# 4m4n5/CLIP-Lite

Hardware: AMD Instinct MI355X
Metric: image-caption pairs/sec (global batch) — ResNet-50+BERT bs1024, 1/2/4/8 MI355X (higher is better)
Workload: dtype bf16; 1 GPU; resnet50 + BERT-base(12L) + JSD-MI heads/priors, per-GPU batch 128, 224x224 images, 30-token captions, dropout 0.1 + prior noise on, clip 10 + SGD(0.9, wd 1e-4) + Lookahead(5, 0.5); global_batch=128, parallelism=dp1

## Files before the change

clip-lite_amd/csrc/conv_patch.hip:

```cpp
#include "igemm_wide.h"
#include "wide_api.h"
#include <type_traits>
#include "stem_bn.h"

using namespace clite;

#ifndef CLITE_PATCH_WGS
#define CLITE_PATCH_WGS 256
#endif

namespace {

constexpr int PC = 64;
constexpr int PIXB = PC * 2;
constexpr int NTAP = 9;
constexpr int WBYTES = NTAP * PC * PIXB;
constexpr int MAXPIX = 344;
constexpr int PBYTES = MAXPIX * PIXB;
constexpr int NPI = MAXPIX / 8;
constexpr int NPW = (NPI + 7) / 8;
constexpr int EPITCH = PC * 4 + 16;
constexpr int HALF = 128;
static_assert(HALF * EPITCH <= PBYTES, "a half of the accumulator tile fits a patch buffer");
static_assert(WBYTES + 2 * PBYTES <= 160 * 1024, "LDS budget");
// ... 265 lines not shown
  a.x = x; a.xbytes = (uint32_t)((size_t)c.N * c.H * c.W * PC * 2);
  a.w = w; a.wbytes = (uint32_t)(NTAP * PC * PC * 2);
  a.N = c.N; a.H = c.H; a.W = c.W; a.R = R;
  a.strips_per_img = (c.H + R - 1) / R;
  a.nstrips = c.N * a.strips_per_img;
  a.flip = dgrad ? 1 : 0;
  const int grid = a.nstrips < CLITE_PATCH_WGS ? a.nstrips : CLITE_PATCH_WGS;
  const int per = (a.nstrips + grid - 1) / grid;
  const int g2 = (a.nstrips + per - 1) / per;
  if (form == 0) hipLaunchKernelGGL(conv3x3_patch_kernel<0>, dim3(g2), dim3(512), 0, st, a, ep, per);
  else hipLaunchKernelGGL(conv3x3_patch_kernel<1>, dim3(g2), dim3(512), 0, st, a, ep, per);
  return (int)hipGetLastError();
}

namespace {

constexpr int WG_DYPIX = 256;
constexpr int WG_XPIX = 376;
constexpr int WG_DYB = WG_DYPIX * PIXB, WG_XB = WG_XPIX * PIXB, WG_STAGE = WG_DYB + WG_XB;
constexpr int WG_NI_DY = WG_DYPIX / 8, WG_NI_X = WG_XPIX / 8;
constexpr int WG_NW_DY = (WG_NI_DY + 7) / 8, WG_NW_X = (WG_NI_X + 7) / 8;
constexpr int WG_OUT = NTAP * PC * PC;
static_assert(2 * WG_STAGE <= 160 * 1024, "LDS budget");

struct WgradPatchArgs {
  const void* dy;
  const void* x;
  uint32_t bytes;
  int N, H, W, R;
  int strips_per_img, nstrips;
  float* ws;
};

DEV int wg_frag_base(int pix0, int x0, int lane) {
  const int x = x0 + 16 * ((lane >> 4) & 1) + 4 * (lane & 3);
  const int pix = pix0 + 8 * (lane >> 5) + ((lane >> 2) & 3);
  const int b = x * 2;
  return pix * PIXB + ((((b >> 6) ^ (pix >> 1)) & 1) << 6) + (b & 63);
}
DEV bf16x8 wg_frag_at(const char* p) {
  const s16x4 lo = lds_read_tr16(p);
  const s16x4 hi = lds_read_tr16(p + 4 * PIXB);
  union { s16x4 v[2]; bf16x8 h; } u;
  u.v[0] = lo; u.v[1] = hi;
  return u.h;
}

__global__ __launch_bounds__(512) void conv3x3_wgrad_patch_kernel(WgradPatchArgs a, int strips_per_wg) {
  __shared__ __attribute__((aligned(1024))) char smem[2 * WG_STAGE];
  const int tid = threadIdx.x;
  const int lane = tid & 63;
  const int wave = wave_uniform(tid >> 6);
  const int W1 = a.W + 1;

  int s_begin = blockIdx.x * strips_per_wg, s_end = s_begin + strips_per_wg;
  if (s_end > a.nstrips) s_end = a.nstrips;

  const rsrc_t rdy = make_rsrc(a.dy, a.bytes), rx = make_rsrc(a.x, a.bytes);
  int d_rel[WG_NW_DY], d_row[WG_NW_DY], x_rel[WG_NW_X], x_row[WG_NW_X];
#pragma unroll
  for (int k = 0; k < WG_NW_DY; ++k) {
    const int i = wave + 8 * k;
    const int pix = i * 8 + (lane >> 3);
    const int oy = pix / W1, ox = pix - oy * W1;
    const int chunk = (lane & 7) ^ (((pix >> 1) & 1) << 2);
    const bool ok = i < WG_NI_DY && ox < a.W && oy < a.R;
    d_row[k] = ok ? oy : -1;
    d_rel[k] = (oy * a.W + ox) * PC + chunk * 8;
  }
#pragma unroll
  for (int k = 0; k < WG_NW_X; ++k) {
    const int i = wave + 8 * k;
    const int pix = i * 8 + (lane >> 3);
    const int pr = pix / W1, pc = pix - pr * W1;
    const int chunk = (lane & 7) ^ (((pix >> 1) & 1) << 2);
    const bool ok = i < WG_NI_X && pc >= 1 && pc <= a.W && pr <= a.R + 1;
    x_row[k] = ok ? pr : -1;
    x_rel[k] = ((pr - 1) * a.W + (pc - 1)) * PC + chunk * 8;
  }
  auto issue = [&](int strip, char* dst) {
// ... 298 lines not shown
```

clip-lite_amd/csrc/gemm_group.hip:

```cpp
#include "igemm_wide.h"
#include "det.h"
#include <string.h>
#include <algorithm>
#include <vector>

using namespace clite;

namespace {

constexpr int GBK = 32;
#ifndef CLITE_GROUP_KCHUNK
#define CLITE_GROUP_KCHUNK 256
#endif
constexpr int KCHUNK = CLITE_GROUP_KCHUNK;

template <class LA, class LB>
struct GroupItem {
  LA la;
  LB lb;
  float* out;
  int ldc, M, N, ktiles, chunk;
  int zeroed;
  const float* row_scale;
  const float* sa;
  const float* sb;
};
struct WgEntry { uint32_t item, tile_m, tile_n, kchunk; };

template <class CFG, class LA, class LB, int NSTAGE>
__global__ __launch_bounds__(256) void igemm_group_kernel(const GroupItem<LA, LB>* __restrict__ items, const WgEntry* __restrict__ map) {
  typedef bf16 T;
  constexpr int BM = CFG::BM, BN = CFG::BN, BK = CFG::BK;
  constexpr int RM = CFG::RM, RN = CFG::RN;
  constexpr int STAGE = LA::BYTES + LB::BYTES;
  constexpr int LOADS_PER_TILE = LA::NI + LB::NI;
  __shared__ __attribute__((aligned(1024))) char smem[NSTAGE * STAGE];

  const int tid = threadIdx.x;
  const int lane = tid & 63;
  const int wave = wave_uniform(tid >> 6);
  const int wm0 = (wave / CFG::WAVES_N) * CFG::WM;
  const int wn0 = (wave % CFG::WAVES_N) * CFG::WN;
  const WgEntry e = map[blockIdx.x];
  if (wave_uniform((int)e.item) < 0) return;
  const GroupItem<LA, LB>& it = items[wave_uniform((int)e.item)];
  const LA la = it.la;
  const LB lb = it.lb;
  const int M = it.M, N = it.N;
  const int m0 = wave_uniform((int)e.tile_m) * BM, n0 = wave_uniform((int)e.tile_n) * BN;
  const int t_begin = wave_uniform((int)e.kchunk) * it.chunk;
  int t_end = t_begin + it.chunk;
  if (t_end > it.ktiles) t_end = it.ktiles;

  typename LA::State sa;
  typename LB::State sb;
  la.init(sa, m0, wave, lane, t_begin);
  lb.init(sb, n0, wave, lane, t_begin);

  f32x16 acc[RM][RN];
#pragma unroll
  for (int i = 0; i < RM; ++i)
#pragma unroll
    for (int j = 0; j < RN; ++j)
#pragma unroll
      for (int r = 0; r < 16; ++r) acc[i][j][r] = 0.f;
  int aoff[RM][BK / 16], boff[RN][BK / 16];
#pragma unroll
  for (int ks = 0; ks < BK / 16; ++ks) {
#pragma unroll
    for (int i = 0; i < RM; ++i) aoff[i][ks] = LA::frag_off(wm0 + i * 32, ks, lane);
#pragma unroll
    for (int j = 0; j < RN; ++j) boff[j][ks] = LB::frag_off(wn0 + j * 32, ks, lane);
  }
#pragma unroll
  for (int pz = 0; pz < NSTAGE - 1; ++pz) {
    if (t_begin + pz < t_end) {
      DmaIssue<LA>::go(la, sa, smem + pz * STAGE, wave, lane, m0);
      DmaIssue<LB>::go(lb, sb, smem + pz * STAGE + LA::BYTES, wave, lane, n0);
// ... 242 lines not shown
    if (t + NSTAGE - 1 < t_end) {
      int nb = buf + NSTAGE - 1; if (nb >= NSTAGE) nb -= NSTAGE;
      WideIssue<LA>::go(la, sa, smem + nb * STAGE, wave, lane, m0);
      WideIssue<LB>::go(lb, sb, smem + nb * STAGE + LA::BYTES, wave, lane, n0);
    }
#pragma unroll
    for (int i = 0; i < RM; ++i)
#pragma unroll
      for (int j = 0; j < RN; ++j) acc[i][j] = mfma32x64_bf8_fp8(alo[i], ahi[i], blo[j], bhi[j], acc[i][j]);
    if (++buf == NSTAGE) buf = 0;
  }
  float* out = it.out;
  const int ldc = it.ldc;
  const float dq = it.sa[1] * it.sb[1];
  const float* rs = it.row_scale;
  const bool single = wave_uniform((int)(it.ktiles <= it.chunk && it.zeroed && !rs));
#pragma unroll
  for (int i = 0; i < RM; ++i)
#pragma unroll
    for (int j = 0; j < RN; ++j) {
      const int col = n0 + wn0 + j * 32 + (lane & 31);
#pragma unroll
      for (int r = 0; r < 16; ++r) {
        const int row = m0 + wm0 + i * 32 + (r & 3) + 8 * (r >> 2) + 4 * (lane >> 5);
        if (row < M && col < N) {
          float* q = out + (size_t)row * ldc + col;
          const float v = (rs ? acc[i][j][r] * rs[row] : acc[i][j][r]) * dq;
          if (single) *q = v; else atomic_add_f32(q, v);
        }
      }
    }
}

struct Plan { int M, N, Ktot, ktiles, chunk, nchunks, tm, tn; };
Plan plan(int M, int N, int Ktot, int BM, int BN, int bk = GBK, int kchunk = KCHUNK) {
  Plan p;
  p.M = M; p.N = N; p.Ktot = Ktot;
  p.ktiles = (Ktot + bk - 1) / bk;
  p.nchunks = (p.ktiles + kchunk - 1) / kchunk;
  p.chunk = (p.ktiles + p.nchunks - 1) / p.nchunks;
  p.nchunks = (p.ktiles + p.chunk - 1) / p.chunk;
  p.tm = (M + BM - 1) / BM; p.tn = (N + BN - 1) / BN;
  return p;
}

FastDiv fastdiv_make(uint32_t d) {
  FastDiv f;
  f.d = d;
  if (d <= 1) { f.mul = 0; f.shift = 0; f.d = 1; return f; }
  uint32_t l = 0;
  while ((1ull << l) < d) ++l;
  f.shift = l;
  f.mul = (uint32_t)((((1ull << l) - d) << 32) / d + 1);
  return f;
}
ConvGeom geom_fwd(const clite_conv& c) {
  ConvGeom g;
  g.H = c.H; g.W = c.W; g.C = c.C;
  g.sN = c.H * c.W * c.C; g.sH = c.W * c.C; g.sW = c.C;
  g.RH = c.Ho; g.RW = c.Wo; g.R = c.R; g.S = c.S; g.stride = c.stride; g.pad = c.pad; g.padw = c.pad;
  g.rows = c.N * c.Ho * c.Wo; g.concat = 0;
  g.div_hw = fastdiv_make(c.Ho * c.Wo);
  g.div_w = fastdiv_make(c.Wo);
  return g;
}

typedef TileCfg<128, 128, GBK, 64, 64> C128;
typedef TileCfg<64, 128, GBK, 64, 32> C64x128;
typedef TileCfg<128, 64, GBK, 32, 64> C128x64;
typedef DmaXCStrided<bf16, 128, GBK> XS128;
typedef DmaXCStrided<bf16, 64, GBK> XS64;
typedef DmaXCGather<bf16, 128, GBK> XG128;
typedef DmaXCGather<bf16, 64, GBK> XG64;
typedef WideCfg<256, 256, 128, 64, 1> W256;
typedef DmaXCStrided<bf16, 256, WIDE_BK, WIDE_NW> WS256;
typedef DmaXCGather<bf16, 256, WIDE_BK, WIDE_NW> WG256;
typedef DmaXCStrided<uint8_t, 256, WIDE_BK, WIDE_NW> FS256;
typedef DmaXCGather<uint8_t, 256, WIDE_BK, WIDE_NW> FG256;
constexpr int WKCHUNK = 128;
template <class CFG> struct GroupStages { static constexpr int n = 3; };
template <> struct GroupStages<W256> { static constexpr int n = 2; };

template <class CFG, class LA, class LB, bool WIDE = false, bool F8 = false>
struct Bucket {
  std::vector<GroupItem<LA, LB>> items;
  std::vector<Plan> plans;
  std::vector<WgEntry> map;
  void add(const LA& la, const LB& lb, float* out, int ldc, const Plan& p, int zeroed, const float* row_scale = nullptr, const float* sa = nullptr,
           const float* sb = nullptr) {
    GroupItem<LA, LB> it;
    it.la = la; it.lb = lb; it.out = out; it.ldc = ldc; it.M = p.M; it.N = p.N; it.ktiles = p.ktiles; it.chunk = p.chunk; it.zeroed = zeroed;
    it.row_scale = row_scale;
    it.sa = sa; it.sb = sb;
    items.push_back(it);
    plans.push_back(p);
  }
  static constexpr uint32_t NO_ITEM = 0xFFFFFFFFu;
  static constexpr int XCDS = 8, BUNDLE = WIDE ? 32 : 64;
  void build_map() {
    std::vector<uint32_t> order(items.size());
    for (uint32_t i = 0; i < order.size(); ++i) order[i] = i;
    std::stable_sort(order.begin(), order.end(), [&](uint32_t a, uint32_t b) { return plans[a].chunk > plans[b].chunk; });
    std::vector<WgEntry> per_xcd[XCDS];
    uint64_t load[XCDS] = {};
    for (uint32_t idx : order) {
      const Plan& p = plans[idx];
      const int tiles = p.tm * p.tn;
      for (int c = 0; c < p.nchunks; ++c) {
        int len = p.chunk;
        if ((c + 1) * p.chunk > p.ktiles) len = p.ktiles - c * p.chunk;
        for (int t0 = 0; t0 < tiles; t0 += BUNDLE) {
          const int t1 = t0 + BUNDLE < tiles ? t0 + BUNDLE : tiles;
          int x = 0;
          for (int k = 1; k < XCDS; ++k)
            if (load[k] < load[x]) x = k;
          for (int t = t0; t < t1; ++t) per_xcd[x].push_back(WgEntry{idx, (uint32_t)(t / p.tn), (uint32_t)(t % p.tn), (uint32_t)c});
          load[x] += (uint64_t)(t1 - t0) * (uint64_t)len;
        }
      }
    }
    size_t longest = 0;
    for (int k = 0; k < XCDS; ++k) longest = per_xcd[k].size() > longest ? per_xcd[k].size() : longest;
    map.assign(longest * XCDS, WgEntry{NO_ITEM, 0, 0, 0});
    for (int k = 0; k < XCDS; ++k)
      for (size_t j = 0; j < per_xcd[k].size(); ++j) map[j * XCDS + k] = per_xcd[k][j];
  }
  size_t n_wgs() const { return map.size(); }
  size_t item_bytes() const { return (items.size() * sizeof(GroupItem<LA, LB>) + 255) / 256 * 256; }
  size_t bytes() const { return item_bytes() + (n_wgs() * sizeof(WgEntry) + 255) / 256 * 256; }
  void stage(char* host, size_t off) {
    if (items.empty()) return;
    memcpy(host + off, items.data(), items.size() * sizeof(GroupItem<LA, LB>));
    memcpy(host + off + item_bytes(), map.data(), map.size() * sizeof(WgEntry));
  }
  int launch(char* dev, size_t off, hipStream_t st) const {
    if (items.empty()) return 0;
    if constexpr (F8)
      hipLaunchKernelGGL((igemm_group_fp8_kernel<CFG, LA, LB, 3>), dim3((unsigned)map.size()), dim3(512), 0, st,
                         (const GroupItem<LA, LB>*)(dev + off), (const WgEntry*)(dev + off + item_bytes()));
    else if constexpr (WIDE)
      hipLaunchKernelGGL((igemm_group_wide_kernel<CFG, LA, LB, GroupStages<CFG>::n>), dim3((unsigned)map.size()), dim3(512), 0, st,
                         (const GroupItem<LA, LB>*)(dev + off), (const WgEntry*)(dev + off + item_bytes()));
    else
      hipLaunchKernelGGL((igemm_group_kernel<CFG, LA, LB, 3>), dim3((unsigned)map.size()), dim3(256), 0, st,
                         (const GroupItem<LA, LB>*)(dev + off), (const WgEntry*)(dev + off + item_bytes()));
    return (int)hipGetLastError();
  }
};

bool fits32(size_t elems, size_t esize) { return elems * esize < 0xF0000000ull; }

}

bool clite_group_wide_enabled();

extern "C" int clite_wgrad_group(int dtype, const clite_wgrad_item* items, int n, void* ws_dev, void* ws_host, uint64_t ws_bytes, void* stream) {
  if (!items || n <= 0) return n == 0 ? 0 : -1;
  hipStream_t st = (hipStream_t)stream;
  if (dtype != CLITE_BF16 || clite::deterministic() || !ws_dev || !ws_host) {
    for (int i = 0; i < n; ++i) {
      const clite_wgrad_item& w = items[i];
      int rc;
      if (w.row_scale || (w.kind & 0xFF) == 2) return -1;
      if ((w.kind & ~(CLITE_WGRAD_NARROW | CLITE_WGRAD_ZEROED | CLITE_WGRAD_SHORTK)) == 0) {
        rc = clite_conv_wgrad(w.a, w.b, &w.cv, w.out, stream);
      } else {
        clite_epilogue ep = {};
        ep.out = w.out; ep.ldc = w.ldc; ep.out_f32 = 1; ep.atomic = 1; ep.alpha = 1.f;
        rc = clite_gemm_tn(w.a, w.lda, w.b, w.ldb, w.M, w.N, w.K, dtype, &ep, stream);
      }
      if (rc) return rc;
    }
    return 0;
  }
  Bucket<C128, XS128, XG128> conv_full;
  Bucket<C64x128, XS64, XG128> conv_fewk;
  Bucket<C128x64, XS128, XG64> conv_fewc;
  Bucket<C128, XS128, XS128> linear;
  Bucket<W256, WS256, WG256, true> conv_w256;
  Bucket<W256, WS256, WS256, true> linear_w256;
  Bucket<W256, FS256, FG256, true, true> conv_f8;
  const bool wide_all = clite_group_wide_enabled();
  for (int i = 0; i < n; ++i) {
    const clite_wgrad_item& w = items[i];
    if (!w.a || !w.b || !w.out) return -1;
    const bool wide = wide_all && !(w.kind & CLITE_WGRAD_NARROW);
    const int zeroed = (w.kind & CLITE_WGRAD_ZEROED) ? 1 : 0;
    const int kind = w.kind & ~(CLITE_WGRAD_NARROW | CLITE_WGRAD_ZEROED | CLITE_WGRAD_SHORTK);
    const int kc = (w.kind & CLITE_WGRAD_SHORTK) ? KCHUNK / 4 : KCHUNK, wkc = (w.kind & CLITE_WGRAD_SHORTK) ? WKCHUNK / 4 : WKCHUNK;
    if (kind == 0) {
      const clite_conv& c = w.cv;
      if (c.dtype != CLITE_BF16 || c.C % 8 || c.K % 8 || (c.R * c.S > 1 && (c.C % 32 || c.K % 32))) return -1;
      if (!fits32((size_t)c.N * c.H * c.W * c.C, 4) || !fits32((size_t)c.N * c.Ho * c.Wo * c.K, 4)) return -1;
      const int P = c.N * c.Ho * c.Wo, Ncols = c.R * c.S * c.C;
      const uint32_t yb = (uint32_t)((size_t)P * c.K * 2), xb = (uint32_t)((size_t)c.N * c.H * c.W * c.C * 2);
      if (wide && c.K >= 256 && Ncols >= 256) conv_w256.add(WS256{w.a, yb, c.K, c.K, P, 1}, WG256{w.b, xb, geom_fwd(c)}, w.out, Ncols, plan(c.K, Ncols, P, 256, 256, WIDE_BK, wkc), zeroed, w.row_scale);
      else if (c.K <= 64) conv_fewk.add(XS64{w.a, yb, c.K, c.K, P, 1}, XG128{w.b, xb, geom_fwd(c)}, w.out, Ncols, plan(c.K, Ncols, P, 64, 128, GBK, kc), zeroed, w.row_scale);
      else if (Ncols <= 64) conv_fewc.add(XS128{w.a, yb, c.K, c.K, P, 1}, XG64{w.b, xb, geom_fwd(c)}, w.out, Ncols, plan(c.K, Ncols, P, 128, 64, GBK, kc), zeroed, w.row_scale);
      else conv_full.add(XS128{w.a, yb, c.K, c.K, P, 1}, XG128{w.b, xb, geom_fwd(c)}, w.out, Ncols, plan(c.K, Ncols, P, 128, 128, GBK, kc), zeroed, w.row_scale);
    } else if (kind == 2) {
      const clite_conv& c = w.cv;
      if (!w.a_scales || !w.b_scales || c.dtype != CLITE_BF16 || c.C % 16 || c.K % 16 || (c.R * c.S > 1 && (c.C % 32 || c.K % 32))) return -1;
      if (!fits32((size_t)c.N * c.H * c.W * c.C, 1) || !fits32((size_t)c.N * c.Ho * c.Wo * c.K, 1)) return -1;
      const int P = c.N * c.Ho * c.Wo, Ncols = c.R * c.S * c.C;
      const uint32_t yb = (uint32_t)((size_t)P * c.K), xb = (uint32_t)((size_t)c.N * c.H * c.W * c.C);
      conv_f8.add(FS256{w.a, yb, c.K, c.K, P, 1}, FG256{w.b, xb, geom_fwd(c)}, w.out, Ncols, plan(c.K, Ncols, P, 256, 256, WIDE_BK, wkc), zeroed, w.row_scale, w.a_scales,
                  w.b_scales);
    } else if (kind == 1) {
      if (w.M <= 0 || w.N <= 0 || w.K <= 0 || w.M % 8 || w.N % 8 || w.lda % 8 || w.ldb % 8 || w.lda < w.M || w.ldb < w.N) return -1;
      if (!fits32((size_t)w.K * w.lda, 4) || !fits32((size_t)w.K * w.ldb, 4)) return -1;
      const uint32_t ab = (uint32_t)((((size_t)w.K - 1) * w.lda + w.M) * 2), bb = (uint32_t)((((size_t)w.K - 1) * w.ldb + w.N) * 2);
      if (wide && w.M >= 256 && w.N >= 256) linear_w256.add(WS256{w.a, ab, w.lda, w.M, w.K, 1}, WS256{w.b, bb, w.ldb, w.N, w.K, 1}, w.out, w.ldc, plan(w.M, w.N, w.K, 256, 256, WIDE_BK, wkc), zeroed, w.row_scale);
      else linear.add(XS128{w.a, ab, w.lda, w.M, w.K, 1}, XS128{w.b, bb, w.ldb, w.N, w.K, 1}, w.out, w.ldc, plan(w.M, w.N, w.K, 128, 128, GBK, kc), zeroed, w.row_scale);
    } else {
      return -1;
    }
  }
  conv_full.build_map(); conv_fewk.build_map(); conv_fewc.build_map(); linear.build_map();
  conv_w256.build_map(); linear_w256.build_map(); conv_f8.build_map();
  const size_t o0 = 0, o1 = o0 + conv_full.bytes(), o2 = o1 + conv_fewk.bytes(), o3 = o2 + conv_fewc.bytes(), o4 = o3 + linear.bytes(),
               o7 = o4 + conv_w256.bytes(), o8 = o7 + linear_w256.bytes(), need = o8 + conv_f8.bytes();
  if (need > ws_bytes) return -2;
  char* host = (char*)ws_host;
  char* dev = (char*)ws_dev;
  conv_full.stage(host, o0); conv_fewk.stage(host, o1); conv_fewc.stage(host, o2); linear.stage(host, o3);
  conv_w256.stage(host, o4); linear_w256.stage(host, o7); conv_f8.stage(host, o8);
  int rc = (int)hipMemcpyAsync(dev, host, need, hipMemcpyHostToDevice, st);
  if (rc) return rc;
  if ((rc = conv_f8.launch(dev, o8, st))) return rc;
  if ((rc = conv_w256.launch(dev, o4, st))) return rc;
  if ((rc = linear_w256.launch(dev, o7, st))) return rc;
  if ((rc = conv_full.launch(dev, o0, st))) return rc;
// ... 11 lines not shown
```

clip-lite_amd/csrc/igemm_dma.h:

```cpp
#ifndef CLITE_IGEMM_DMA_H
#define CLITE_IGEMM_DMA_H
#ifndef CLITE_ABLATE
#define CLITE_ABLATE 0
#endif
#ifndef CLITE_STAMP
#define CLITE_STAMP 0
#endif
#if CLITE_STAMP
__device__ unsigned long long clite_dbg[8 * 65536];
#define EPI_STAMP(i) do { if (threadIdx.x == 0 && blockIdx.x < 65536) clite_dbg[blockIdx.x * 8 + (i)] = __builtin_amdgcn_s_memrealtime(); } while (0)
#define STAMP(i) do { if (threadIdx.x == 0 && blockIdx.x < 65536) clite_dbg[blockIdx.x * 8 + (i)] = __builtin_amdgcn_s_memrealtime(); } while (0)
__shared__ unsigned long long clite_ph[8];
#define PHASE(i) do { if (threadIdx.x == 0) { unsigned long long n_ = __builtin_amdgcn_s_memrealtime(); clite_ph[i] += n_ - clite_ph[7]; clite_ph[7] = n_; } } while (0)
#define BN_EPI_PHASE(i) PHASE(i)
#else
#define STAMP(i) do {} while (0)
#define PHASE(i) do {} while (0)
#endif
#include "igemm.h"

namespace clite {

template <typename T, int ROWS, int BK, bool DGRAD>
struct DmaKC {
// ... 193 lines not shown
      int krow = (wave * NI + j) * RPI + lane / CPR;
      int c = (lane % CPR) ^ (xc_seg_xor<ROWB>(krow) << 2);
      int x = x0 + c * EPC;
      int rs = x / g.C;
      int ci = x - rs * g.C;
      st.r[j] = rs / g.S;
      st.s[j] = rs - st.r[j] * g.S;
      st.krow[j] = krow;
      st.xoff[j] = x < g.R * g.S * g.C ? ci : -1;
    }
    st.p0 = t_begin * BK;
  }
  DEV void issue(State& st, char* lds, int wave, int, int) const {
#pragma unroll
    for (int j = 0; j < NI; ++j) {
      int p = st.p0 + st.krow[j];
      bool v = st.xoff[j] >= 0 && p < g.rows;
      uint32_t n = fd_div(p, g.div_hw);
      uint32_t rem = p - n * g.div_hw.d;
      uint32_t ho = fd_div(rem, g.div_w);
      uint32_t wo = rem - ho * g.div_w.d;
      int hi = (int)ho * g.stride - g.pad + st.r[j];
      int wi = (int)wo * g.stride - g.padw + st.s[j];
      v = v && (unsigned)hi < (unsigned)g.H && (unsigned)wi < (unsigned)g.W;
      uint32_t off = v ? (uint32_t)((int)n * g.sN + hi * g.sH + wi * g.sW + st.xoff[j]) * (uint32_t)sizeof(T) : OOB_OFF;
      buf_load16_lds(st.rs_, off, lds + (wave * NI + j) * 1024);
    }
    st.p0 += BK;
  }
  DEV static int frag_off(int x0, int ks, int lane) { return L::frag_off(x0, ks, lane); }
  DEV static bf16x8 frag_at(const char* p) { return L::frag_at(p); }
  DEV static float frag32(const char* lds, int x0, int kk, int lane) { return L::frag32(lds, x0, kk, lane); }
  DEV static void frag8_f32(const char* lds, int x0, int lane, float (&v)[8]) { L::frag8_f32(lds, x0, lane, v); }
};

template <class L> struct DmaIssue {
  DEV static void go(const L& l, typename L::State& st, char* lds, int wave, int lane, int x0) { l.issue(st, lds, wave, lane, x0); }
};
template <typename T, int ROWS, int BK, bool D> struct DmaIssue<DmaKC<T, ROWS, BK, D>> {
  typedef DmaKC<T, ROWS, BK, D> L;
  DEV static void go(const L& l, typename L::State& st, char* lds, int wave, int, int) { l.issue(st, lds, wave); }
};

DEV void split_bf16x3(const float (&v)[8], bf16x8& hi, bf16x8& lo) {
#pragma unroll
  for (int e = 0; e < 8; ++e) {
    const bf16 h = f2bf(v[e]);
    hi[e] = h;
    lo[e] = f2bf(v[e] - bf2f(h));
  }
}
template <class CFG, class LA, class LB>
DEV void mma_tile_f32_split(const char* abuf, const char* bbuf, int wm0, int wn0, int lane, f32x16 (&acc)[CFG::RM][CFG::RN]) {
  constexpr int RM = CFG::RM, RN = CFG::RN;
  bf16x8 ah[RM], al[RM], bh[RN], bl[RN];
#pragma unroll
  for (int i = 0; i < RM; ++i) {
    float v[8];
    LA::frag8_f32(abuf, wm0 + i * 32, lane, v);
    split_bf16x3(v, ah[i], al[i]);
  }
#pragma unroll
  for (int j = 0; j < RN; ++j) {
    float v[8];
    LB::frag8_f32(bbuf, wn0 + j * 32, lane, v);
    split_bf16x3(v, bh[j], bl[j]);
// ... 530 lines not shown
```

clip-lite_amd/hip.py:

```python
import ctypes as C
import os

import torch

_HERE = os.path.dirname(os.path.abspath(__file__))
LIB_PATH = os.environ.get("CLITE_HIP_LIB") or os.path.join(_HERE, "lib", "libclite_hip.so")
ABI_VERSION = 12

BF16, F32 = 0, 1
ACT_NONE, ACT_RELU, ACT_GELU, ACT_TANH = 0, 1, 2, 3
DACT_RELU, DACT_GELU, DACT_TANH = 1, 2, 3
SEED_INDIRECT = 0x80000000

TORCH_DTYPE = {BF16: torch.bfloat16, F32: torch.float32}


class Epilogue(C.Structure):
    _fields_ = [
        ("out", C.c_void_p), ("ldc", C.c_int32), ("out_f32", C.c_int32), ("atomic", C.c_int32),
        ("alpha", C.c_float), ("bias", C.c_void_p), ("act", C.c_int32), ("preact", C.c_void_p),
        ("dact_aux", C.c_void_p), ("dact", C.c_int32), ("drop_p", C.c_float), ("drop_seed", C.c_uint64),
        ("drop_site", C.c_uint32), ("residual", C.c_void_p), ("colsum", C.c_void_p),
        ("colsum_replicas", C.c_int32), ("colsum_stride", C.c_int32), ("colsum_rows", C.c_int32),
        ("bn_y", C.c_void_p), ("bn_stats", C.c_void_p), ("bn_replicas", C.c_int32), ("bn_rstride", C.c_int32),
# ... 382 lines not shown
    if rc == 1:
        conv_wgrad(dy, x, cv, dw)
    else:
        check(rc, "conv_wgrad_patch")


import collections
_inflight_groups = collections.deque()
_ws_pool = []


KCHUNK_TILES = 256


class WgradGroup:

    wide = True

    def __init__(self, dt, workspace=None, zeroed=False):
        self.dt, self.items, self.extra, self.keep, self.wgs = dt, [], [], [], 0
        self.post = []
        self.kflags = 0x200 if zeroed else 0
        self.ws_dev, self.ws_host = workspace if workspace is not None else (None, None)

    @staticmethod
    def alloc_workspace(device, nbytes=4 << 20):
        return torch.empty(nbytes, dtype=torch.uint8, device=device), torch.empty(nbytes, dtype=torch.uint8).pin_memory()

    @staticmethod
    def _wgs(M, N, K, bm=128, bn=128):
        kt = (K + 31) // 32
        return ((M + bm - 1) // bm) * ((N + bn - 1) // bn) * ((kt + KCHUNK_TILES - 1) // KCHUNK_TILES)

    patch = False

    def conv(self, dy, x, cv, dw, row_scale=None, short_k=False):
        if row_scale is None and self.patch and self.wide and conv_wgrad_patch_applies(cv) and not is_deterministic():
            self.keep += [dy, x, dw]
            self.extra.append(lambda: conv_wgrad_patch(dy, x, cv, dw))
            return
        it = WgradItem()
        it.kind, it.a, it.b, it.out, it.cv = (0 if self.wide else 0x100) | self.kflags | (0x400 if short_k else 0), p(dy), p(x), p(dw), cv
        it.row_scale = p(row_scale)
        self.items.append(it)
        self.keep += [dy, x, dw, row_scale]
        ncols = cv.R * cv.S * cv.C
        self.wgs += self._wgs(cv.K, ncols, cv.N * cv.Ho * cv.Wo, 64 if cv.K <= 64 else 128, 64 if ncols <= 64 else 128) * (4 if short_k else 1)

    def conv_fp8(self, dy8, x8, cv, dw):
        it = WgradItem()
        it.kind, it.a, it.b, it.out, it.cv = 2 | self.kflags, p(dy8.q), p(x8.q), p(dw), cv
        it.a_scales, it.b_scales = p(dy8.scales), p(x8.scales)
        self.items.append(it)
        self.keep += [dy8.q, x8.q, dy8.scales, x8.scales, dw]
        self.wgs += self._wgs(cv.K, cv.R * cv.S * cv.C, cv.N * cv.Ho * cv.Wo, 256, 256)

    def linear(self, A, B, M, N, K, out, lda=None, ldb=None, ldc=None):
        it = WgradItem()
        it.kind, it.a, it.b, it.out = (1 if self.wide else 0x101) | self.kflags, p(A), p(B), p(out)
        it.M, it.N, it.K, it.lda, it.ldb, it.ldc = M, N, K, lda or M, ldb or N, ldc or N
        self.items.append(it)
        self.keep += [A, B, out]
        self.wgs += self._wgs(M, N, K)

    def call(self, fn):
        self.extra.append(fn)

    def after(self, fn):
        self.post.append(fn)

    def launch_extras(self):
        for fn in self.extra:
            fn()

    def launch(self, extras=True):
# ... 369 lines not shown
```

include/clite.h:

```cpp
#ifndef CLITE_H
#define CLITE_H
#include <stdint.h>

#ifdef __cplusplus
extern "C" {
#endif

#define CLITE_ABI_VERSION 12
int clite_abi_version(void);

int clite_set_deterministic(int on);
int clite_get_deterministic(void);

int clite_set_f32_split(int on);
int clite_get_f32_split(void);

int clite_set_tile_policy(int policy);

enum { CLITE_BF16 = 0, CLITE_F32 = 1 };

#define CLITE_SEED_INDIRECT 0x80000000u

enum { CLITE_ACT_NONE = 0, CLITE_ACT_RELU = 1, CLITE_ACT_GELU = 2, CLITE_ACT_TANH = 3 };

// ... 24 lines not shown
  int32_t mask_after_residual;
  const uint8_t* relu_bits;
  float* splitk_ws;
  int32_t residual_subsample;
  uint8_t* fp8_out;
  const float* fp8_scale;
  float* fp8_amax;
} clite_epilogue;

typedef struct clite_conv {
  int32_t dtype;
  int32_t N, H, W, C;
  int32_t K, R, S;
  int32_t stride, pad;
  int32_t Ho, Wo;
} clite_conv;

int clite_gemm_nt(const void* A, int lda, const void* B, int ldb, int M, int N, int K, int dtype, const clite_epilogue* ep, void* stream);
int clite_gemm_nn(const void* A, int lda, const void* B, int ldb, int M, int N, int K, int dtype, const clite_epilogue* ep, void* stream);
int clite_gemm_tn(const void* A, int lda, const void* B, int ldb, int M, int N, int K, int dtype, const clite_epilogue* ep, void* stream);

int clite_conv_fwd(const void* x, const void* w, const clite_conv* cv, const clite_epilogue* ep, void* stream);
int clite_conv_dgrad(const void* dy, const void* w, const clite_conv* cv, const clite_epilogue* ep, void* stream);
int clite_conv_dgrad_s2class(const void* dy, const void* wsub, const clite_conv* cv, int ph, int pw, const clite_epilogue* ep, void* stream);
int clite_conv_dgrad_wt(const void* dy, const void* wt, const clite_conv* cv, const clite_epilogue* ep, void* stream);
int clite_conv_dgrad_s2class_wt(const void* dy, const void* wtsub, const clite_conv* cv, int ph, int pw, const clite_epilogue* ep, void* stream);
int clite_conv_wgrad(const void* dy, const void* x, const clite_conv* cv, float* dw, void* stream);
int clite_conv_wgrad_patch_workspace(uint64_t* nbytes);
int clite_conv_wgrad_patch(const void* dy, const void* x, const clite_conv* cv, float* dw, void* ws, uint64_t ws_bytes, void* stream);

#define CLITE_WGRAD_NARROW 0x100
#define CLITE_WGRAD_ZEROED 0x200
#define CLITE_WGRAD_SHORTK 0x400
typedef struct clite_wgrad_item {
  int32_t kind;
  const void* a;
  const void* b;
  float* out;
  clite_conv cv;
  int32_t M, N, K, lda, ldb, ldc;
  const float* a_scales;
  const float* b_scales;
  const float* row_scale;
} clite_wgrad_item;
int clite_wgrad_group(int dtype, const clite_wgrad_item* items, int n, void* ws_dev, void* ws_host, uint64_t ws_bytes, void* stream);
int clite_wgrad_group_workspace(int n_items, int64_t total_workgroups, uint64_t* bytes);

typedef struct clite_transpose_item {
  uint64_t src_off, dst_off;
  uint32_t rows, cols, src_ld, dst_ld, batch, src_bstride, dst_bstride, first_tile;
} clite_transpose_item;
int clite_transpose_weights(const void* src, void* dst, const clite_transpose_item* items_dev, int n_items, uint32_t total_tiles, void* stream);

int clite_fp8_quantize(int dtype, const void* x, uint64_t n, float* amax, float* scales, void* out_fp8, void* stream);
int clite_gemm_nt_fp8(const void* A8, int lda, const void* B8, int ldb, int M, int N, int K, const float* a_scales, const float* b_scales,
                      const clite_epilogue* ep, void* stream);
int clite_conv_fwd_fp8(const void* x8, const void* w8, const clite_conv* cv, const float* x_scales, const float* w_scales,
                       const clite_epilogue* ep, void* stream);
int clite_conv_dgrad_fp8(const void* dy8, const void* wt8, const clite_conv* cv, const float* dy_scales, const float* w_scales,
                         const clite_epilogue* ep, void* stream);
#define CLITE_FP8_AMAX_REPLICAS 16
#define CLITE_FP8_AMAX_STRIDE 32
int clite_fp8_scale_update(float* amax, float* scales, int n, void* stream);
typedef struct clite_fp8_item {
  uint64_t offset, numel;
} clite_fp8_item;
// ... 174 lines not shown
```

Baseline: 8809 pairs/s.

## Add patch-tap form for 64-channel 3x3 wgrad inside the grouped GEMM launch

Adds a second member form to the grouped wgrad kernel. For bf16 3x3 stride-1 convolutions with 64 input and 64 output channels, it stages strips of dy and a haloed x patch in LDS once and computes three taps per workgroup from shared fragments, instead of running the generic implicit-GEMM gather. The host scheduler now weights work by a per-form cost when sorting and balancing across XCDs, and picks the number of strip chunks from the ratio of operand bytes to atomic output traffic. This replaces the old separately launched patch kernel path, which was disabled. It trades redundant gather loads for more atomic adds into the small 64x576 output and for extra branching and a larger item struct in the shared kernel.

```diff
diff --git a/clip-lite_amd/csrc/conv_patch.hip b/clip-lite_amd/csrc/conv_patch.hip
--- a/clip-lite_amd/csrc/conv_patch.hip
+++ b/clip-lite_amd/csrc/conv_patch.hip
@@ -321,20 +321,6 @@
   float* ws;
 };
 
-DEV int wg_frag_base(int pix0, int x0, int lane) {
-  const int x = x0 + 16 * ((lane >> 4) & 1) + 4 * (lane & 3);
-  const int pix = pix0 + 8 * (lane >> 5) + ((lane >> 2) & 3);
-  const int b = x * 2;
-  return pix * PIXB + ((((b >> 6) ^ (pix >> 1)) & 1) << 6) + (b & 63);
-}
-DEV bf16x8 wg_frag_at(const char* p) {
-  const s16x4 lo = lds_read_tr16(p);
-  const s16x4 hi = lds_read_tr16(p + 4 * PIXB);
-  union { s16x4 v[2]; bf16x8 h; } u;
-  u.v[0] = lo; u.v[1] = hi;
-  return u.h;
-}
-
 __global__ __launch_bounds__(512) void conv3x3_wgrad_patch_kernel(WgradPatchArgs a, int strips_per_wg) {
   __shared__ __attribute__((aligned(1024))) char smem[2 * WG_STAGE];
   const int tid = threadIdx.x;
diff --git a/clip-lite_amd/csrc/gemm_group.hip b/clip-lite_amd/csrc/gemm_group.hip
--- a/clip-lite_amd/csrc/gemm_group.hip
+++ b/clip-lite_amd/csrc/gemm_group.hip
@@ -13,6 +13,9 @@
 #define CLITE_GROUP_KCHUNK 256
 #endif
 constexpr int KCHUNK = CLITE_GROUP_KCHUNK;
+#ifndef CLITE_PT_ATOMIC_SHARE
+#define CLITE_PT_ATOMIC_SHARE 20
+#endif
 
 template <class LA, class LB>
 struct GroupItem {
@@ -24,16 +27,68 @@
   const float* row_scale;
   const float* sa;
   const float* sb;
+  int form;
+  DmaPatchTap<4> pt;
 };
 struct WgEntry { uint32_t item, tile_m, tile_n, kchunk; };
 
-template <class CFG, class LA, class LB, int NSTAGE>
+template <class ITEM>
+DEV void patch_tap_member(const ITEM& it, const WgEntry& e, char* smem, int wave, int lane) {
+  const DmaPatchTap<4> pt = it.pt;
+  const int r = wave_uniform((int)e.tile_n);
+  const int s_begin = wave_uniform((int)e.kchunk) * it.chunk;
+  int s_end = s_begin + it.chunk;
+  if (s_end > it.ktiles) s_end = it.ktiles;
+  typename DmaPatchTap<4>::State st;
+  pt.init(st, r, wave, lane);
+  const int coh = wave >> 1, cih = wave & 1;
+  const int oa = wg_frag_base(0, 32 * coh, lane);
+  const int ob0 = wg_frag_base(0, 32 * cih, lane), ob1 = wg_frag_base(1, 32 * cih, lane), ob2 = wg_frag_base(2, 32 * cih, lane);
+  f32x16 acc0, acc1, acc2;
+#pragma unroll
+  for (int q = 0; q < 16; ++q) { acc0[q] = 0.f; acc1[q] = 0.f; acc2[q] = 0.f; }
+  if (s_begin < s_end) pt.issue(st, s_begin, smem, wave);
+  for (int strip = s_begin; strip < s_end; ++strip) {
+    const int cur = (strip - s_begin) & 1;
+    wait_vmcnt<0>();
+    lds_barrier();
+    if (strip + 1 < s_end) pt.issue(st, strip + 1, smem + (cur ^ 1) * PT_STAGE, wave);
+    const char* dyi = smem + cur * PT_STAGE;
+    const char* xi = dyi + PT_DYB;
+#pragma unroll
+    for (int ks = 0; ks < PT_DYPIX / 16; ++ks) {
+      const bf16x8 fa = wg_frag_at(dyi + oa + ks * 16 * 128);
+      const bf16x8 f0 = wg_frag_at(xi + ob0 + ks * 16 * 128), f1 = wg_frag_at(xi + ob1 + ks * 16 * 128), f2 = wg_frag_at(xi + ob2 + ks * 16 * 128);
+      acc0 = mfma32_bf16(fa, f0, acc0);
+      acc1 = mfma32_bf16(fa, f1, acc1);
+      acc2 = mfma32_bf16(fa, f2, acc2);
+    }
+  }
+  float* out = it.out;
+  const int ldc = it.ldc;
+  const float* rs = it.row_scale;
+  const bool single = wave_uniform((int)(it.ktiles <= it.chunk && it.zeroed && !rs));
+  auto put = [&](const f32x16& v, int s) {
+    const int col = (r * 3 + s) * 64 + 32 * cih + (lane & 31);
+#pragma unroll
+    for (int q = 0; q < 16; ++q) {
+      const int row = 32 * coh + (q & 3) + 8 * (q >> 2) + 4 * (lane >> 5);
+      float* p = out + (size_t)row * ldc + col;
+      const float val = rs ? v[q] * rs[row] : v[q];
+      if (single) *p = val; else atomic_add_f32(p, val);
+    }
+  };
+  put(acc0, 0); put(acc1, 1); put(acc2, 2);
+}
+
+template <class CFG, class LA, class LB, int NSTAGE, bool PT = false>
 __global__ __launch_bounds__(256) void igemm_group_kernel(const GroupItem<LA, LB>* __restrict__ items, const WgEntry* __restrict__ map) {
   typedef bf16 T;
   constexpr int BM = CFG::BM, BN = CFG::BN, BK = CFG::BK;
   constexpr int RM = CFG::RM, RN = CFG::RN;
   constexpr int STAGE = LA::BYTES + LB::BYTES;
   constexpr int LOADS_PER_TILE = LA::NI + LB::NI;
+  static_assert(!PT || 2 * PT_STAGE <= NSTAGE * STAGE, "the patch-tap form's two stages fit the ring of the tile form");
   __shared__ __attribute__((aligned(1024))) char smem[NSTAGE * STAGE];
 
   const int tid = threadIdx.x;
@@ -44,6 +99,12 @@
   const WgEntry e = map[blockIdx.x];
   if (wave_uniform((int)e.item) < 0) return;
   const GroupItem<LA, LB>& it = items[wave_uniform((int)e.item)];
+  if constexpr (PT) {
+    if (wave_uniform(it.form) == 1) {
+      patch_tap_member(it, e, smem, wave, lane);
+      return;
+    }
+  }
   const LA la = it.la;
   const LB lb = it.lb;
   const int M = it.M, N = it.N;
@@ -352,10 +413,11 @@
     }
 }
 
-struct Plan { int M, N, Ktot, ktiles, chunk, nchunks, tm, tn; };
-Plan plan(int M, int N, int Ktot, int BM, int BN, int bk = GBK, int kchunk = KCHUNK) {
+constexpr int COST_1 = 4, COST_GATHER3 = COST_1, COST_PATCH = 6;
+struct Plan { int M, N, Ktot, ktiles, chunk, nchunks, tm, tn, cost; };
+Plan plan(int M, int N, int Ktot, int BM, int BN, int bk = GBK, int kchunk = KCHUNK, int cost = COST_1) {
   Plan p;
-  p.M = M; p.N = N; p.Ktot = Ktot;
+  p.M = M; p.N = N; p.Ktot = Ktot; p.cost = cost;
   p.ktiles = (Ktot + bk - 1) / bk;
   p.nchunks = (p.ktiles + kchunk - 1) / kchunk;
   p.chunk = (p.ktiles + p.nchunks - 1) / p.nchunks;
@@ -401,7 +463,7 @@
 template <class CFG> struct GroupStages { static constexpr int n = 3; };
 template <> struct GroupStages<W256> { static constexpr int n = 2; };
 
-template <class CFG, class LA, class LB, bool WIDE = false, bool F8 = false>
+template <class CFG, class LA, class LB, bool WIDE = false, bool F8 = false, bool PT = false>
 struct Bucket {
   std::vector<GroupItem<LA, LB>> items;
   std::vector<Plan> plans;
@@ -412,6 +474,33 @@
     it.la = la; it.lb = lb; it.out = out; it.ldc = ldc; it.M = p.M; it.N = p.N; it.ktiles = p.ktiles; it.chunk = p.chunk; it.zeroed = zeroed;
     it.row_scale = row_scale;
     it.sa = sa; it.sb = sb;
+    it.form = 0;
+    it.pt = DmaPatchTap<4>{};
+    items.push_back(it);
+    plans.push_back(p);
+  }
+  void add_patch(const void* dy, const void* x, const clite_conv& c, float* out, const Plan& gather, int zeroed, const float* row_scale) {
+    static_assert(PT, "patch-tap members need the PT instantiation");
+    GroupItem<LA, LB> it = {};
+    it.pt.dy = dy; it.pt.x = x;
+    it.pt.dybytes = it.pt.xbytes = (uint32_t)((size_t)c.N * c.H * c.W * 64 * 2);
+    it.pt.H = c.H; it.pt.W = c.W;
+    it.pt.R = PT_DYPIX / (c.W + 1) < c.H ? PT_DYPIX / (c.W + 1) : c.H;
+    it.pt.strips_per_img = (c.H + it.pt.R - 1) / it.pt.R;
+    const int nstrips = c.N * it.pt.strips_per_img;
+    const double op_bytes = 2.0 * it.pt.dybytes, out_bytes = 64.0 * 9 * 64 * 4;
+    long nch = (long)(op_bytes / (CLITE_PT_ATOMIC_SHARE * out_bytes));
+    const long cap = (long)gather.tm * gather.tn * gather.nchunks / 3;
+    if (nch > cap) nch = cap;
+    if (nch > nstrips) nch = nstrips;
+    if (nch < 1) nch = 1;
+    Plan p = {};
+    p.M = 64; p.N = 9 * 64; p.Ktot = nstrips; p.ktiles = nstrips; p.cost = COST_PATCH;
+    p.chunk = (int)((nstrips + nch - 1) / nch);
+    p.nchunks = (nstrips + p.chunk - 1) / p.chunk;
+    p.tm = 1; p.tn = 3;
+    it.out = out; it.ldc = 9 * 64; it.M = 64; it.N = 9 * 64; it.ktiles = nstrips; it.chunk = p.chunk; it.zeroed = zeroed; it.row_scale = row_scale;
+    it.form = 1;
     items.push_back(it);
     plans.push_back(p);
   }
@@ -420,7 +509,8 @@
   void build_map() {
     std::vector<uint32_t> order(items.size());
     for (uint32_t i = 0; i < order.size(); ++i) order[i] = i;
-    std::stable_sort(order.begin(), order.end(), [&](uint32_t a, uint32_t b) { return plans[a].chunk > plans[b].chunk; });
+    std::stable_sort(order.begin(), order.end(),
+                     [&](uint32_t a, uint32_t b) { return (int64_t)plans[a].chunk * plans[a].cost > (int64_t)plans[b].chunk * plans[b].cost; });
     std::vector<WgEntry> per_xcd[XCDS];
     uint64_t load[XCDS] = {};
     for (uint32_t idx : order) {
@@ -435,7 +525,7 @@
           for (int k = 1; k < XCDS; ++k)
             if (load[k] < load[x]) x = k;
           for (int t = t0; t < t1; ++t) per_xcd[x].push_back(WgEntry{idx, (uint32_t)(t / p.tn), (uint32_t)(t % p.tn), (uint32_t)c});
-          load[x] += (uint64_t)(t1 - t0) * (uint64_t)len;
+          load[x] += (uint64_t)(t1 - t0) * (uint64_t)len * (uint64_t)p.cost;
         }
       }
     }
@@ -462,13 +552,18 @@
       hipLaunchKernelGGL((igemm_group_wide_kernel<CFG, LA, LB, GroupStages<CFG>::n>), dim3((unsigned)map.size()), dim3(512), 0, st,
                          (const GroupItem<LA, LB>*)(dev + off), (const WgEntry*)(dev + off + item_bytes()));
     else
-      hipLaunchKernelGGL((igemm_group_kernel<CFG, LA, LB, 3>), dim3((unsigned)map.size()), dim3(256), 0, st,
+      hipLaunchKernelGGL((igemm_group_kernel<CFG, LA, LB, 3, PT>), dim3((unsigned)map.size()), dim3(256), 0, st,
                          (const GroupItem<LA, LB>*)(dev + off), (const WgEntry*)(dev + off + item_bytes()));
     return (int)hipGetLastError();
   }
 };
 
 bool fits32(size_t elems, size_t esize) { return elems * esize < 0xF0000000ull; }
+
+bool patch_tap_applies(const clite_conv& c) {
+  return c.dtype == CLITE_BF16 && c.C == 64 && c.K == 64 && c.R == 3 && c.S == 3 && c.stride == 1 && c.pad == 1 && c.Ho == c.H && c.Wo == c.W &&
+         c.W + 1 <= PT_DYPIX;
+}
 
 }
 
@@ -482,7 +577,7 @@
       const clite_wgrad_item& w = items[i];
       int rc;
       if (w.row_scale || (w.kind & 0xFF) == 2) return -1;
-      if ((w.kind & ~(CLITE_WGRAD_NARROW | CLITE_WGRAD_ZEROED | CLITE_WGRAD_SHORTK)) == 0) {
+      if ((w.kind & ~(CLITE_WGRAD_NARROW | CLITE_WGRAD_ZEROED | CLITE_WGRAD_SHORTK | CLITE_WGRAD_PATCH)) == 0) {
         rc = clite_conv_wgrad(w.a, w.b, &w.cv, w.out, stream);
       } else {
         clite_epilogue ep = {};
@@ -494,7 +589,7 @@
     return 0;
   }
   Bucket<C128, XS128, XG128> conv_full;
-  Bucket<C64x128, XS64, XG128> conv_fewk;
+  Bucket<C64x128, XS64, XG128, false, false, true> conv_fewk;
   Bucket<C128x64, XS128, XG64> conv_fewc;
   Bucket<C128, XS128, XS128> linear;
   Bucket<W256, WS256, WG256, true> conv_w256;
@@ -506,7 +601,7 @@
     if (!w.a || !w.b || !w.out) return -1;
     const bool wide = wide_all && !(w.kind & CLITE_WGRAD_NARROW);
     const int zeroed = (w.kind & CLITE_WGRAD_ZEROED) ? 1 : 0;
-    const int kind = w.kind & ~(CLITE_WGRAD_NARROW | CLITE_WGRAD_ZEROED | CLITE_WGRAD_SHORTK);
+    const int kind = w.kind & ~(CLITE_WGRAD_NARROW | CLITE_WGRAD_ZEROED | CLITE_WGRAD_SHORTK | CLITE_WGRAD_PATCH);
     const int kc = (w.kind & CLITE_WGRAD_SHORTK) ? KCHUNK / 4 : KCHUNK, wkc = (w.kind & CLITE_WGRAD_SHORTK) ? WKCHUNK / 4 : WKCHUNK;
     if (kind == 0) {
       const clite_conv& c = w.cv;
@@ -514,10 +609,13 @@
       if (!fits32((size_t)c.N * c.H * c.W * c.C, 4) || !fits32((size_t)c.N * c.Ho * c.Wo * c.K, 4)) return -1;
       const int P = c.N * c.Ho * c.Wo, Ncols = c.R * c.S * c.C;
       const uint32_t yb = (uint32_t)((size_t)P * c.K * 2), xb = (uint32_t)((size_t)c.N * c.H * c.W * c.C * 2);
-      if (wide && c.K >= 256 && Ncols >= 256) conv_w256.add(WS256{w.a, yb, c.K, c.K, P, 1}, WG256{w.b, xb, geom_fwd(c)}, w.out, Ncols, plan(c.K, Ncols, P, 256, 256, WIDE_BK, wkc), zeroed, w.row_scale);
-      else if (c.K <= 64) conv_fewk.add(XS64{w.a, yb, c.K, c.K, P, 1}, XG128{w.b, xb, geom_fwd(c)}, w.out, Ncols, plan(c.K, Ncols, P, 64, 128, GBK, kc), zeroed, w.row_scale);
-      else if (Ncols <= 64) conv_fewc.add(XS128{w.a, yb, c.K, c.K, P, 1}, XG64{w.b, xb, geom_fwd(c)}, w.out, Ncols, plan(c.K, Ncols, P, 128, 64, GBK, kc), zeroed, w.row_scale);
-      else conv_full.add(XS128{w.a, yb, c.K, c.K, P, 1}, XG128{w.b, xb, geom_fwd(c)}, w.out, Ncols, plan(c.K, Ncols, P, 128, 128, GBK, kc), zeroed, w.row_scale);
+      const int cost = c.R * c.S > 1 ? COST_GATHER3 : COST_1;
+      if ((w.kind & CLITE_WGRAD_PATCH) && patch_tap_applies(c))
+        conv_fewk.add_patch(w.a, w.b, c, w.out, plan(c.K, Ncols, P, 64, 128, GBK, kc), zeroed, w.row_scale);
+      else if (wide && c.K >= 256 && Ncols >= 256) conv_w256.add(WS256{w.a, yb, c.K, c.K, P, 1}, WG256{w.b, xb, geom_fwd(c)}, w.out, Ncols, plan(c.K, Ncols, P, 256, 256, WIDE_BK, wkc), zeroed, w.row_scale);
+      else if (c.K <= 64) conv_fewk.add(XS64{w.a, yb, c.K, c.K, P, 1}, XG128{w.b, xb, geom_fwd(c)}, w.out, Ncols, plan(c.K, Ncols, P, 64, 128, GBK, kc, cost), zeroed, w.row_scale);
+      else if (Ncols <= 64) conv_fewc.add(XS128{w.a, yb, c.K, c.K, P, 1}, XG64{w.b, xb, geom_fwd(c)}, w.out, Ncols, plan(c.K, Ncols, P, 128, 64, GBK, kc, cost), zeroed, w.row_scale);
+      else conv_full.add(XS128{w.a, yb, c.K, c.K, P, 1}, XG128{w.b, xb, geom_fwd(c)}, w.out, Ncols, plan(c.K, Ncols, P, 128, 128, GBK, kc, cost), zeroed, w.row_scale);
     } else if (kind == 2) {
       const clite_conv& c = w.cv;
       if (!w.a_scales || !w.b_scales || c.dtype != CLITE_BF16 || c.C % 16 || c.K % 16 || (c.R * c.S > 1 && (c.C % 32 || c.K % 32))) return -1;
diff --git a/clip-lite_amd/csrc/igemm_dma.h b/clip-lite_amd/csrc/igemm_dma.h
--- a/clip-lite_amd/csrc/igemm_dma.h
+++ b/clip-lite_amd/csrc/igemm_dma.h
@@ -249,6 +249,78 @@
   DEV static bf16x8 frag_at(const char* p) { return L::frag_at(p); }
   DEV static float frag32(const char* lds, int x0, int kk, int lane) { return L::frag32(lds, x0, kk, lane); }
   DEV static void frag8_f32(const char* lds, int x0, int lane, float (&v)[8]) { L::frag8_f32(lds, x0, lane, v); }
+};
+
+DEV int wg_frag_base(int pix0, int x0, int lane) {
+  const int x = x0 + 16 * ((lane >> 4) & 1) + 4 * (lane & 3);
+  const int pix = pix0 + 8 * (lane >> 5) + ((lane >> 2) & 3);
+  const int b = x * 2;
+  return pix * 128 + ((((b >> 6) ^ (pix >> 1)) & 1) << 6) + (b & 63);
+}
+DEV bf16x8 wg_frag_at(const char* p) {
+  const s16x4 lo = lds_read_tr16(p);
+  const s16x4 hi = lds_read_tr16(p + 4 * 128);
+  union { s16x4 v[2]; bf16x8 h; } u;
+  u.v[0] = lo; u.v[1] = hi;
+  return u.h;
+}
+
+constexpr int PT_DYPIX = 64;
+constexpr int PT_XPIX = 72;
+constexpr int PT_DYB = PT_DYPIX * 128, PT_XB = PT_XPIX * 128, PT_STAGE = PT_DYB + PT_XB;
+constexpr int PT_NI_DY = PT_DYPIX / 8, PT_NI = PT_NI_DY + PT_XPIX / 8;
+template <int NW>
+struct DmaPatchTap {
+  static constexpr int NPW = (PT_NI + NW - 1) / NW;
+  const void* dy;
+  const void* x;
+  uint32_t dybytes, xbytes;
+  int H, W, R, strips_per_img;
+
+  struct State {
+    rsrc_t rdy, rx;
+    int rel[NPW];
+    int row[NPW];
+  };
+  DEV void init(State& st, int r, int wave, int lane) const {
+    st.rdy = make_rsrc(dy, dybytes);
+    st.rx = make_rsrc(x, xbytes);
+    const int W1 = W + 1;
+#pragma unroll
+    for (int k = 0; k < NPW; ++k) {
+      const int i = wave + NW * k;
+      if (i < PT_NI_DY) {
+        const int pix = i * 8 + (lane >> 3);
+        const int oy = pix / W1, ox = pix - oy * W1;
+        const int chunk = (lane & 7) ^ (((pix >> 1) & 1) << 2);
+        st.row[k] = ox < W && oy < R ? oy : -1;
+        st.rel[k] = (oy * W + ox) * 64 + chunk * 8;
+      } else {
+        const int j = (i - PT_NI_DY) * 8 + (lane >> 3);
+        const int q = r * W1 + j;
+        const int pr = q / W1, pc = q - pr * W1;
+        const int chunk = (lane & 7) ^ (((j >> 1) & 1) << 2);
+        st.row[k] = i < PT_NI && pc >= 1 && pr <= R + 1 ? pr : -1;
+        st.rel[k] = ((pr - 1) * W + (pc - 1)) * 64 + chunk * 8;
+      }
+    }
+  }
+  DEV void issue(const State& st, int strip, char* dst, int wave) const {
+    const int n = strip / strips_per_img;
+    const int y0 = (strip - n * strips_per_img) * R;
+    const int base = (n * H + y0) * W * 64;
+#pragma unroll
+    for (int k = 0; k < NPW; ++k) {
+      const int i = wave + NW * k;
+      if (i < PT_NI_DY) {
+        const bool v = st.row[k] >= 0 && y0 + st.row[k] < H;
+        buf_load16_lds_nt(st.rdy, v ? (uint32_t)((base + st.rel[k]) * 2) : OOB_OFF, dst + i * 1024);
+      } else if (i < PT_NI) {
+        const bool v = st.row[k] >= 0 && (unsigned)(y0 + st.row[k] - 1) < (unsigned)H;
+        buf_load16_lds_nt(st.rx, v ? (uint32_t)((base + st.rel[k]) * 2) : OOB_OFF, dst + i * 1024);
+      }
+    }
+  }
 };
 
 template <class L> struct DmaIssue {
diff --git a/clip-lite_amd/hip.py b/clip-lite_amd/hip.py
--- a/clip-lite_amd/hip.py
+++ b/clip-lite_amd/hip.py
@@ -438,15 +438,13 @@
         kt = (K + 31) // 32
         return ((M + bm - 1) // bm) * ((N + bn - 1) // bn) * ((kt + KCHUNK_TILES - 1) // KCHUNK_TILES)
 
-    patch = False
+    patch_tap = True
 
     def conv(self, dy, x, cv, dw, row_scale=None, short_k=False):
-        if row_scale is None and self.patch and self.wide and conv_wgrad_patch_applies(cv) and not is_deterministic():
-            self.keep += [dy, x, dw]
-            self.extra.append(lambda: conv_wgrad_patch(dy, x, cv, dw))
-            return
         it = WgradItem()
         it.kind, it.a, it.b, it.out, it.cv = (0 if self.wide else 0x100) | self.kflags | (0x400 if short_k else 0), p(dy), p(x), p(dw), cv
+        if self.patch_tap:
+            it.kind |= 0x800
         it.row_scale = p(row_scale)
         self.items.append(it)
         self.keep += [dy, x, dw, row_scale]
diff --git a/include/clite.h b/include/clite.h
--- a/include/clite.h
+++ b/include/clite.h
@@ -80,6 +80,7 @@
 #define CLITE_WGRAD_NARROW 0x100
 #define CLITE_WGRAD_ZEROED 0x200
 #define CLITE_WGRAD_SHORTK 0x400
+#define CLITE_WGRAD_PATCH 0x800
 typedef struct clite_wgrad_item {
   int32_t kind;
   const void* a;
```

Result: no change. 8783 pairs/s, median of 2 (-0.3%).
